# davidesantangelo/krep

Measured on NVIDIA H100. Metric: GB/s scanned (HBM-resident corpus), higher is better.
Workload: dtype u8

## Files before the change

krep_b200/csrc/scan_count.cu:

```cuda
#include <algorithm>
#include "engine.h"
#include "line_rec.cuh"
#include "lit_filters.cuh"

namespace kb {

struct CountDev
{
    LitDevParams p;
    uint64_t own_end;
    uint32_t part_groups, n_parts;
    uint32_t exact;
    uint32_t tail;
    LineRec *recs;
};

struct PartState
{
    uint32_t lines = 0;
    bool has_hit = false, first_open = false, pending = false, seen_nl = false;
    uint64_t covered_to = 0;
};

__device__ __noinline__ unsigned verify_exact_call(const LitDevParams &p, long long cand) { return verify_exact(p, cand); }

__device__ __noinline__ bool scan_for_newline(const LitDevParams &p, uint64_t lo, uint64_t hi)
{
    const uint32_t lane = threadIdx.x & 31;
    if (hi > p.avail_len) hi = p.avail_len;
    for (uint64_t base = lo & ~15ull; base < hi; base += 512)
    {
        const uint64_t unit = base + 16ull * lane;
        uint32_t nm = 0;
        if (unit < hi && unit + 16 > lo)
        {
            if (unit + 16 <= p.avail_len) nm = nl_mask16(__ldg(reinterpret_cast<const uint4 *>(p.text + unit)));
            else
                for (uint64_t q = unit; q < p.avail_len; q++) nm |= (p.text[q] == '\n' ? 1u : 0u) << (uint32_t)(q - unit);
            nm &= range_mask16(unit, lo, hi);
        }
        if (__any_sync(0xffffffffu, nm != 0)) return true;
    }
    return false;
}

__device__ __forceinline__ void settle(const LitDevParams &p, PartState &S, uint64_t upto)
{
    if (S.covered_to < upto && (S.pending || (!S.has_hit && !S.seen_nl)))
        if (scan_for_newline(p, S.covered_to, upto))
        {
            S.pending = false;
            S.seen_nl = true;
        }
}

__device__ __forceinline__ void account(PartState &S, uint32_t hm, uint32_t nm)
{
    const uint32_t lane = threadIdx.x & 31;
    const bool has_nl = nm != 0;
    const uint32_t fnl = has_nl ? (uint32_t)__ffs(nm) - 1 : 0, lnl = has_nl ? 31u - (uint32_t)__clz(nm) : 0;
    const bool f = has_nl && (hm & ((1u << fnl) - 1u)) != 0;
    const bool l = has_nl && ((hm >> lnl) >> 1) != 0;
    uint32_t inner = 0;
    if (__popc(nm) >= 2)
    {
        uint32_t prev = fnl, rest = nm & (nm - 1);
        while (rest)
        {
            const uint32_t nx = (uint32_t)__ffs(rest) - 1;
            if (hm & (((1u << nx) - 1u) & ~((2u << prev) - 1u))) inner++;
            prev = nx;
            rest &= rest - 1;
        }
    }
    const uint32_t A = __ballot_sync(0xffffffffu, has_nl), T = __ballot_sync(0xffffffffu, !has_nl && hm != 0);
    const uint32_t F = __ballot_sync(0xffffffffu, f), Lm = __ballot_sync(0xffffffffu, l);
    uint32_t innersum = 0;
    if (__ballot_sync(0xffffffffu, inner != 0)) innersum = __reduce_add_sync(0xffffffffu, inner);
    if (A == 0)
    {
        if (T)
        {
            if (!S.pending)
            {
                S.lines++;
                if (!S.has_hit && !S.seen_nl) S.first_open = true;
            }
            S.pending = true;
            S.has_hit = true;
        }
        return;
    }
    const uint32_t j1 = (uint32_t)__ffs(A) - 1, jr = 31u - (uint32_t)__clz(A);
    if ((T & ((1u << j1) - 1u)) || ((F >> j1) & 1u))
    {
        if (!S.pending)
        {
            S.lines++;
            if (!S.has_hit && !S.seen_nl) S.first_open = true;
        }
        S.has_hit = true;
    }
    S.pending = false;
    S.seen_nl = true;
    bool gap = false;
    if (has_nl && lane != j1)
    {
        const uint32_t below = A & ((1u << lane) - 1u);
        const uint32_t pj = 31u - (uint32_t)__clz(below);
        const uint32_t between = ((1u << lane) - 1u) & ~((2u << pj) - 1u);
        gap = ((Lm >> pj) & 1u) || (T & between) || f;
    }
    const uint32_t G = __ballot_sync(0xffffffffu, gap);
    S.lines += (uint32_t)__popc(G) + innersum;
    if (G || innersum) S.has_hit = true;
    if (((Lm >> jr) & 1u) || ((T >> jr) >> 1))
    {
        S.lines++;
        S.has_hit = true;
        S.pending = true;
    }
}

__device__ __forceinline__ uint64_t pack_state(const PartState &S)
{
    return (uint64_t)S.lines | ((uint64_t)((S.has_hit ? 1u : 0u) | (S.first_open ? 2u : 0u) | (S.pending ? 4u : 0u) | (S.seen_nl ? 8u : 0u)) << 32);
}
__device__ __forceinline__ void unpack_state(uint64_t k, PartState &S)
{
    S.lines = (uint32_t)k;
    const uint32_t f = (uint32_t)(k >> 32);
    S.has_hit = f & 1u;
    S.first_open = f & 2u;
    S.pending = f & 4u;
    S.seen_nl = f & 8u;
}
__device__ __noinline__ uint64_t account_call(uint64_t packed, uint32_t hm, uint32_t nm)
{
    PartState S;
    unpack_state(packed, S);
    account(S, hm, nm);
    return pack_state(S);
}

template <bool WINDOW>
__device__ __noinline__ uint32_t hit_mask16(const CountDev &D, uint64_t unit, const uint4 &v, uint32_t nx)
{
    const LitDevParams &p = D.p;
    const uint32_t w[5] = {v.x, v.y, v.z, v.w, nx};
    uint32_t hm = 0;
    if (WINDOW)
    {
        const uint32_t mask = p.fold & p.win_mask, k0 = p.K[0];
#pragma unroll
        for (int k = 0; k < 4; k++)
#pragma unroll
            for (int r = 0; r < 4; r++)
            {
                const uint32_t win = r == 0 ? w[k] : __funnelshift_r(w[k], w[k + 1], 8 * r);
                if ((win & mask) == k0)
                {
                    const uint64_t st = unit + 4 * k + r;
                    const bool ok = D.exact ? (st >= p.own_begin && st < p.own_end && st + p.m <= p.avail_len)
                                            : verify_exact_call(p, (long long)st) != 0;
                    if (ok) hm |= 1u << (4 * k + r);
                }
            }
    }
    else
    {
#pragma unroll
        for (int k = 0; k < 4; k++)
#pragma unroll
            for (int d = 0; d < 4; d++)
                if ((w[k] & p.fold) == p.K[d] && verify_exact_call(p, (long long)(unit + 4 * k) - d)) hm |= 1u << (4 * k);
    }
    return hm;
}

__device__ __noinline__ PartState count_tail(const CountDev &D, PartState S, uint64_t cov, uint64_t nl_lo, uint64_t nl_hi, bool window)
{
    const LitDevParams &p = D.p;
    const uint32_t lane = threadIdx.x & 31;
    if (p.avail_len < p.emit_len && cov >= nl_hi) return S;
    const uint64_t last_start = p.avail_len >= p.emit_len ? p.avail_len - p.emit_len : 0;
    uint64_t end = nl_hi > last_start + 1 ? nl_hi : last_start + 1;
    if (!window && end < cov + 1) end = cov + 1;
    for (uint64_t base = cov; base < end; base += 32)
    {
        settle(p, S, base > nl_lo ? base : nl_lo);
        const uint64_t q = base + lane;
        uint32_t hm = 0, nm = 0;
        if (q < end)
        {
            if (p.avail_len >= p.emit_len && q >= p.tail_start && q <= last_start && verify_exact(p, (long long)q)) hm = 1;
            if (!window && q == cov && p.avail_len >= p.emit_len)
                for (uint64_t s = p.tail_start; s < cov && s <= last_start; s++)
                    if (verify_exact(p, (long long)s)) hm = 1;
            if (q >= nl_lo && q < nl_hi && q < p.avail_len && p.text[q] == '\n') nm = 1;
            if (nm) hm = 0;
        }
        account(S, hm, nm);
        S.covered_to = base + 32;
    }
    return S;
}

#ifndef KREP_B200_COUNT_MINB
#define KREP_B200_COUNT_MINB 3
#endif
template <bool WINDOW, bool FOLD, bool MASKED>
__global__ void __launch_bounds__(256, KREP_B200_COUNT_MINB) k_count_lines(const __grid_constant__ CountDev D)
{
    const LitDevParams &p = D.p;
    const uint4 *__restrict__ t4 = reinterpret_cast<const uint4 *>(p.text);
    const uint32_t lane = threadIdx.x & 31;
    const uint32_t warp_global = (blockIdx.x * blockDim.x + threadIdx.x) >> 5, total_warps = (gridDim.x * blockDim.x) >> 5;
    const uint32_t k0 = p.K[0], k1 = p.K[1], k2 = p.K[2], k3 = p.K[3], fold = p.fold, mask = p.win_mask;
    const uint32_t c1 = p.mulc[0], c2 = p.mulc[1], c3 = p.mulc[2];
    for (uint32_t pi = warp_global; pi < D.n_parts; pi += total_warps)
    {
        const uint64_t ga = p.group_begin + (uint64_t)pi * D.part_groups;
        uint64_t gb = ga + D.part_groups;
        if (gb > p.group_end) gb = p.group_end;
        const bool last_part = pi + 1 == D.n_parts;
        const uint64_t nl_lo = ga * 16 > p.own_begin ? ga * 16 : p.own_begin;
        const uint64_t nl_hi = (last_part || gb * 16 > D.own_end) ? D.own_end : gb * 16;
        PartState S;
        S.covered_to = nl_lo;
        for (uint64_t g = ga; g < gb; g += 128)
        {
            uint4 v[4];
            uint32_t nx[4];
            bool ok[4];
#pragma unroll
            for (int u = 0; u < 4; u++)
            {
                const uint64_t gi = g + 32 * u + lane;
                ok[u] = gi < gb;
                v[u] = ok[u] ? ld_stream(t4 + gi) : make_uint4(0u, 0u, 0u, 0u);
                nx[u] = 0;
                if (WINDOW && ok[u] && (lane == 31 || gi + 1 >= gb)) nx[u] = __ldg(reinterpret_cast<const uint32_t *>(t4 + gi + 1));
            }
            uint32_t cand = 0;
#pragma unroll
            for (int u = 0; u < 4; u++)
            {
                bool h;
                if (WINDOW)
                {
                    const uint32_t nb = __shfl_down_sync(0xffffffffu, v[u].x, 1);
                    if (!(lane == 31 || g + 32 * u + lane + 1 >= gb)) nx[u] = nb;
                    h = hit_vec_w<FOLD, MASKED>(v[u], nx[u], fold, mask, k0, c1, c2, c3);
                }
                else
                    h = hit_vec<FOLD>(v[u], fold, k0, k1, k2, k3);
                cand |= (h && ok[u]) ? (1u << u) : 0u;
            }
            const uint32_t any = __reduce_or_sync(0xffffffffu, cand);
            if (any)
            {
                const uint64_t tile_lo = g * 16;
                settle(p, S, tile_lo > nl_lo ? tile_lo : nl_lo);
                const bool inside = tile_lo >= nl_lo && tile_lo + 2048 <= nl_hi;
                uint64_t st = pack_state(S);
#pragma unroll
                for (int u = 0; u < 4; u++)
                {
                    const uint64_t unit = tile_lo + 512ull * u + 16ull * lane;
                    uint32_t hm = 0, nm = 0;
                    if (ok[u])
                    {
                        if ((cand >> u) & 1u) hm = hit_mask16<WINDOW>(D, unit, v[u], nx[u]);
                        nm = nl_mask16(v[u]);
                        if (!inside) nm &= range_mask16(unit, nl_lo, nl_hi);
                    }
                    st = account_call(st, hm, nm);
                }
                unpack_state(st, S);
                S.covered_to = tile_lo + 2048;
            }
        }
        if (last_part && D.tail) S = count_tail(D, S, gb * 16, nl_lo, nl_hi, WINDOW);
        uint32_t flags = 0;
        if (S.has_hit)
        {
            if (S.pending && S.covered_to < nl_hi && scan_for_newline(p, S.covered_to, nl_hi)) S.pending = false;
            flags = LR_HAS_HIT | (S.first_open ? LR_FIRST_OPEN : 0u) | (S.pending ? LR_LAST_PENDING : 0u) | LR_HAS_NL;
        }
        else
        {
            const bool nl = S.seen_nl || (S.covered_to < nl_hi && scan_for_newline(p, S.covered_to, nl_hi));
            flags = nl ? LR_HAS_NL : 0u;
        }
        if (lane == 0) D.recs[pi] = LineRec{S.lines, flags};
    }
}

__global__ void __launch_bounds__(1024) k_count_finish(const LineRec *recs, uint32_t n, uint64_t *d_out, uint64_t *h_out)
{
    __shared__ uint64_t s_lines[1024];
    __shared__ uint32_t s_flags[1024];
    const uint32_t per = (n + blockDim.x - 1) / blockDim.x;
    const uint32_t a = threadIdx.x * per, b = a + per < n ? a + per : n;
    uint64_t lines = 0;
    uint32_t flags = 0;
    for (uint32_t i = a; i < b; i++) append_rec(lines, flags, recs[i].lines, recs[i].flags);
    s_lines[threadIdx.x] = lines;
    s_flags[threadIdx.x] = flags;
    __syncthreads();
    if (threadIdx.x == 0)
    {
        lines = 0;
        flags = 0;
        for (uint32_t t = 0; t < blockDim.x; t++) append_rec(lines, flags, s_lines[t], s_flags[t]);
        d_out[0] = lines;
        d_out[1] = flags;
        h_out[0] = lines;
        h_out[1] = flags;
    }
}

#define CKC(call)                                                                                  \
    do                                                                                             \
    {                                                                                              \
        cudaError_t e_ = (call);                                                                   \
        if (e_ != cudaSuccess)                                                                     \
        {                                                                                          \
            set_error(-2, "CUDA error %s at %s:%d (%s)", cudaGetErrorName(e_), __FILE__, __LINE__, \
                      cudaGetErrorString(e_));                                                     \
            return -2;                                                                             \
        }                                                                                          \
    } while (0)

bool count_lines_eligible(const Plan *plan, const search_params_t *P, int algo)
{
    if (!P->count_lines_mode || plan->is_regex || plan->whole_word == 2) return false;
    if (plan->is_ac)
    {
        for (const std::string &s : plan->patterns)
            if (s.find('\n') != std::string::npos) return false;
        return true;
    }
    if (plan->emit_len != plan->m) return false;
    if (plan->pattern.find('\n') != std::string::npos) return false;
    return algo == KREP_B200_ALGO_BMH || algo == KREP_B200_ALGO_KMP || algo == KREP_B200_ALGO_MEMCHR ||
           algo == KREP_B200_ALGO_MEMCHR_SHORT || algo == KREP_B200_ALGO_SSE42;
}

int ensure_line_out(DevCtx &E, uint64_t n)
{
    if (n <= E.line_out_cap) return 0;
    CKC(cudaDeviceSynchronize());
    cudaFree(E.d_line_out);
    cudaFreeHost(E.h_line_out);
    E.d_line_out = nullptr;
    E.h_line_out = nullptr;
    E.line_out_cap = 0;
    uint64_t cap = 64;
    while (cap < n) cap *= 2;
    CKC(cudaMalloc(&E.d_line_out, cap * 2 * sizeof(uint64_t)));
    CKC(cudaHostAlloc(&E.h_line_out, cap * 2 * sizeof(uint64_t), cudaHostAllocMapped | cudaHostAllocPortable));
    E.line_out_cap = cap;
    return 0;
}

int launch_count_lines(DevCtx &E, const Plan *plan, const krep_b200_shard_t *sh, cudaStream_t stream, uint64_t index)
{
    if (((uintptr_t)sh->d_text & 15) != 0)
    {
        set_error(-3, "shard text pointer must be 16-byte aligned");
        return -3;
    }
    const PlanDev *pd = plan_on_device(plan, E);
    if (!pd) return -2;
    if (ensure_line_out(E, index + 1) != 0) return -2;
    if (plan->is_ac)
    {
        const int slot = set_count_slot(E);
        const int rc = set_count_begin(E, plan, sh, stream, slot);
        return rc != 0 ? rc : set_count_end(E, plan, sh, stream, slot, index);
    }
    CountDev D;
    memset(&D, 0, sizeof D);
    LitDevParams &p = D.p;
    const uint64_t own_end = sh->own_end < sh->avail_len ? sh->own_end : sh->avail_len;
    p.text = (const uint8_t *)sh->d_text;
    p.avail_len = sh->avail_len;
    p.own_begin = sh->own_begin;
    p.own_end = own_end;
    p.global_offset = sh->global_offset;
    p.prev_byte = sh->prev_byte;
    p.next_byte = sh->next_byte;
    uint64_t total_groups;
    const bool window = plan->filter == FILTER_WINDOW4;
    if (!window)
    {
        total_groups = sh->avail_len / 16;
        p.tail_start = total_groups ? total_groups * 16 - 3 : 0;
    }
    else
    {
        total_groups = sh->avail_len >= 20 ? (sh->avail_len - 20) / 16 + 1 : 0;
        p.tail_start = total_groups * 16;
    }
    p.group_begin = sh->own_begin / 16;
    p.group_end = (own_end + 2) / 16 + 1;
    D.tail = p.group_end > total_groups ? 1u : 0u;
    if (p.group_end > total_groups) p.group_end = total_groups;
    if (p.group_begin > p.group_end) p.group_begin = p.group_end;
    p.m = plan->m;
    p.emit_len = plan->emit_len;
    for (int d = 0; d < 4; d++) p.K[d] = plan->K[d];
    p.fold = plan->fold;
    p.win_mask = plan->win_mask;
    p.mulc[0] = 1u << 24;
    p.mulc[1] = 1u << 16;
    p.mulc[2] = 1u << 8;
    p.pat_val = pd->d_pat_val;
    p.pat_mask = pd->d_pat_mask;
    p.whole_word = plan->whole_word;
    D.own_end = own_end;
    {
        bool letters = true;
        for (unsigned char ch : plan->pattern) letters &= is_alpha_c(ch);
        D.exact = (window && plan->m <= 4 && plan->whole_word == 0 && (plan->case_sensitive || letters)) ? 1u : 0u;
    }
    const uint64_t groups = p.group_end - p.group_begin;
    const char *v = getenv("KREP_B200_COUNT_PART_KB");
    const uint32_t kb_ = v && atoi(v) > 0 ? (uint32_t)atoi(v) : 64;
    uint64_t part = std::max<uint32_t>(128, kb_ * 64 / 128 * 128);
    const uint64_t max_parts = 1u << 18;
    if ((groups + part - 1) / part > max_parts) part = ((groups + max_parts - 1) / max_parts + 127) / 128 * 128;
    D.part_groups = (uint32_t)part;
    D.n_parts = (uint32_t)std::max<uint64_t>((groups + part - 1) / part, 1);
    if (D.n_parts > E.line_recs_cap)
    {
        CKC(cudaStreamSynchronize(stream));
        cudaFree(E.d_line_recs);
        E.d_line_recs = nullptr;
        E.line_recs_cap = 0;
        const uint64_t cap = std::max<uint64_t>(D.n_parts, 1u << 16);
        CKC(cudaMalloc(&E.d_line_recs, cap * sizeof(LineRec)));
        E.line_recs_cap = cap;
    }
    D.recs = (LineRec *)E.d_line_recs;
    const bool folded = plan->fold != 0xFFFFFFFFu, masked = plan->win_mask != 0xFFFFFFFFu;
    const uint64_t want_blocks = ((uint64_t)D.n_parts + 7) / 8;
    const unsigned grid = (unsigned)std::min<uint64_t>(want_blocks, (uint64_t)E.sm_count * KREP_B200_COUNT_MINB);
    if (!window)
    {
        if (folded) k_count_lines<false, true, false><<<grid, 256, 0, stream>>>(D);
        else k_count_lines<false, false, false><<<grid, 256, 0, stream>>>(D);
    }
    else if (folded)
    {
        if (masked) k_count_lines<true, true, true><<<grid, 256, 0, stream>>>(D);
        else k_count_lines<true, true, false><<<grid, 256, 0, stream>>>(D);
    }
    else
    {
        if (masked) k_count_lines<true, false, true><<<grid, 256, 0, stream>>>(D);
        else k_count_lines<true, false, false><<<grid, 256, 0, stream>>>(D);
    }
    CKC(cudaGetLastError());
    k_count_finish<<<1, 1024, 0, stream>>>(D.recs, D.n_parts, E.d_line_out + 2 * index, E.h_line_out + 2 * index);
    CKC(cudaGetLastError());
    count_launch(2);
    return 0;
}

uint64_t combine_line_records(const uint64_t *recs, size_t n)
{
    uint64_t lines = 0;
    uint32_t flags = 0;
    for (size_t i = 0; i < n; i++) append_rec(lines, flags, recs[2 * i], (uint32_t)recs[2 * i + 1]);
    return lines;
}

}
```

Baseline: 3124.

## Stage count-kernel tiles through cp.async shared-memory ring with per-lane line records

Rewrites the line-counting kernel so each warp streams 2 KB tiles through a 4-stage cp.async shared-memory ring, and each lane handles 64 contiguous bytes instead of strided 16-byte units. The sequential warp-wide account/settle state machine and the separate newline rescans are replaced by per-lane bitmask line records combined with a shuffle-based append_rec reduction. The special tail pass goes away because the last tile is zero-padded. Blocks shrink to 4 warps and the occupancy hint rises to 4. The aim is to hide HBM latency and cut serial per-tile bookkeeping, at the cost of shared-memory footprint and more complex boundary handling.

```diff
diff --git a/krep_b200/csrc/scan_count.cu b/krep_b200/csrc/scan_count.cu
--- a/krep_b200/csrc/scan_count.cu
+++ b/krep_b200/csrc/scan_count.cu
@@ -11,290 +11,211 @@
     uint64_t own_end;
     uint32_t part_groups, n_parts;
     uint32_t exact;
-    uint32_t tail;
     LineRec *recs;
 };
 
-struct PartState
-{
-    uint32_t lines = 0;
-    bool has_hit = false, first_open = false, pending = false, seen_nl = false;
-    uint64_t covered_to = 0;
-};
-
-__device__ __noinline__ unsigned verify_exact_call(const LitDevParams &p, long long cand) { return verify_exact(p, cand); }
-
-__device__ __noinline__ bool scan_for_newline(const LitDevParams &p, uint64_t lo, uint64_t hi)
-{
-    const uint32_t lane = threadIdx.x & 31;
-    if (hi > p.avail_len) hi = p.avail_len;
-    for (uint64_t base = lo & ~15ull; base < hi; base += 512)
-    {
-        const uint64_t unit = base + 16ull * lane;
-        uint32_t nm = 0;
-        if (unit < hi && unit + 16 > lo)
+constexpr uint32_t COUNT_WARPS = 4;
+constexpr uint32_t COUNT_STAGES = 4;
+constexpr uint32_t COUNT_STAGE_BYTES = 2048 + 16;
+#ifndef KREP_B200_COUNT_MINB
+#define KREP_B200_COUNT_MINB 4
+#endif
+
+template <uint32_t UNITS>
+__device__ __forceinline__ void stage_tile(uint32_t s_dst, const uint8_t *text, uint64_t avail, uint64_t pos, uint32_t lane)
+{
+#pragma unroll
+    for (uint32_t i = 0; i < (UNITS + 31) / 32; i++)
+    {
+        const uint32_t u = lane + 32 * i;
+        if (u >= UNITS) break;
+        const uint64_t b = pos + 16ull * u;
+        const uint32_t n = b >= avail ? 0u : (avail - b >= 16 ? 16u : (uint32_t)(avail - b));
+        const uint8_t *src = n ? text + b : text;
+        asm volatile("cp.async.cg.shared.global [%0], [%1], 16, %2;" ::"r"(s_dst + 16u * u), "l"(src), "r"(n) : "memory");
+    }
+    asm volatile("cp.async.commit_group;" ::: "memory");
+}
+
+__device__ __forceinline__ uint64_t umin64(uint64_t a, uint64_t b) { return a < b ? a : b; }
+
+__device__ __forceinline__ uint64_t range_mask64(uint64_t base, uint64_t lo, uint64_t hi)
+{
+    uint64_t m = ~0ull;
+    if (base < lo) m = lo - base >= 64 ? 0ull : m << (uint32_t)(lo - base);
+    if (base + 64 > hi) m = hi <= base ? 0ull : m & (~0ull >> (uint32_t)(64 - (hi - base)));
+    return m;
+}
+
+template <bool WINDOW>
+__device__ __forceinline__ uint32_t cand16(const LitDevParams &p, const uint4 &v, uint32_t nx)
+{
+    const uint32_t w[5] = {v.x, v.y, v.z, v.w, nx};
+    uint32_t c = 0;
+#pragma unroll
+    for (int k = 0; k < 4; k++)
+#pragma unroll
+        for (int r = 0; r < 4; r++)
         {
-            if (unit + 16 <= p.avail_len) nm = nl_mask16(__ldg(reinterpret_cast<const uint4 *>(p.text + unit)));
+            bool h;
+            if (WINDOW)
+            {
+                const uint32_t win = r == 0 ? w[k] : __funnelshift_r(w[k], w[k + 1], 8 * r);
+                h = (win & (p.fold & p.win_mask)) == p.K[0];
+            }
             else
-                for (uint64_t q = unit; q < p.avail_len; q++) nm |= (p.text[q] == '\n' ? 1u : 0u) << (uint32_t)(q - unit);
-            nm &= range_mask16(unit, lo, hi);
+                h = (w[k] & p.fold) == p.K[r];
+            c |= (h ? 1u : 0u) << (4 * k + r);
         }
-        if (__any_sync(0xffffffffu, nm != 0)) return true;
-    }
-    return false;
-}
-
-__device__ __forceinline__ void settle(const LitDevParams &p, PartState &S, uint64_t upto)
-{
-    if (S.covered_to < upto && (S.pending || (!S.has_hit && !S.seen_nl)))
-        if (scan_for_newline(p, S.covered_to, upto))
-        {
-            S.pending = false;
-            S.seen_nl = true;
-        }
-}
-
-__device__ __forceinline__ void account(PartState &S, uint32_t hm, uint32_t nm)
-{
-    const uint32_t lane = threadIdx.x & 31;
-    const bool has_nl = nm != 0;
-    const uint32_t fnl = has_nl ? (uint32_t)__ffs(nm) - 1 : 0, lnl = has_nl ? 31u - (uint32_t)__clz(nm) : 0;
-    const bool f = has_nl && (hm & ((1u << fnl) - 1u)) != 0;
-    const bool l = has_nl && ((hm >> lnl) >> 1) != 0;
-    uint32_t inner = 0;
-    if (__popc(nm) >= 2)
-    {
-        uint32_t prev = fnl, rest = nm & (nm - 1);
-        while (rest)
-        {
-            const uint32_t nx = (uint32_t)__ffs(rest) - 1;
-            if (hm & (((1u << nx) - 1u) & ~((2u << prev) - 1u))) inner++;
-            prev = nx;
-            rest &= rest - 1;
-        }
-    }
-    const uint32_t A = __ballot_sync(0xffffffffu, has_nl), T = __ballot_sync(0xffffffffu, !has_nl && hm != 0);
-    const uint32_t F = __ballot_sync(0xffffffffu, f), Lm = __ballot_sync(0xffffffffu, l);
-    uint32_t innersum = 0;
-    if (__ballot_sync(0xffffffffu, inner != 0)) innersum = __reduce_add_sync(0xffffffffu, inner);
-    if (A == 0)
-    {
-        if (T)
-        {
-            if (!S.pending)
-            {
-                S.lines++;
-                if (!S.has_hit && !S.seen_nl) S.first_open = true;
-            }
-            S.pending = true;
-            S.has_hit = true;
-        }
-        return;
-    }
-    const uint32_t j1 = (uint32_t)__ffs(A) - 1, jr = 31u - (uint32_t)__clz(A);
-    if ((T & ((1u << j1) - 1u)) || ((F >> j1) & 1u))
-    {
-        if (!S.pending)
-        {
-            S.lines++;
-            if (!S.has_hit && !S.seen_nl) S.first_open = true;
-        }
-        S.has_hit = true;
-    }
-    S.pending = false;
-    S.seen_nl = true;
-    bool gap = false;
-    if (has_nl && lane != j1)
-    {
-        const uint32_t below = A & ((1u << lane) - 1u);
-        const uint32_t pj = 31u - (uint32_t)__clz(below);
-        const uint32_t between = ((1u << lane) - 1u) & ~((2u << pj) - 1u);
-        gap = ((Lm >> pj) & 1u) || (T & between) || f;
-    }
-    const uint32_t G = __ballot_sync(0xffffffffu, gap);
-    S.lines += (uint32_t)__popc(G) + innersum;
-    if (G || innersum) S.has_hit = true;
-    if (((Lm >> jr) & 1u) || ((T >> jr) >> 1))
-    {
-        S.lines++;
-        S.has_hit = true;
-        S.pending = true;
-    }
-}
-
-__device__ __forceinline__ uint64_t pack_state(const PartState &S)
-{
-    return (uint64_t)S.lines | ((uint64_t)((S.has_hit ? 1u : 0u) | (S.first_open ? 2u : 0u) | (S.pending ? 4u : 0u) | (S.seen_nl ? 8u : 0u)) << 32);
-}
-__device__ __forceinline__ void unpack_state(uint64_t k, PartState &S)
-{
-    S.lines = (uint32_t)k;
-    const uint32_t f = (uint32_t)(k >> 32);
-    S.has_hit = f & 1u;
-    S.first_open = f & 2u;
-    S.pending = f & 4u;
-    S.seen_nl = f & 8u;
-}
-__device__ __noinline__ uint64_t account_call(uint64_t packed, uint32_t hm, uint32_t nm)
-{
-    PartState S;
-    unpack_state(packed, S);
-    account(S, hm, nm);
-    return pack_state(S);
-}
-
-template <bool WINDOW>
-__device__ __noinline__ uint32_t hit_mask16(const CountDev &D, uint64_t unit, const uint4 &v, uint32_t nx)
-{
+    return c;
+}
+
+__device__ __forceinline__ void lane_record(uint64_t H, uint64_t N, uint32_t &lines, uint32_t &flags)
+{
+    lines = 0;
+    flags = N ? LR_HAS_NL : 0u;
+    if (H)
+    {
+        const uint64_t t = ~N + H;
+        const bool open = t < H;
+        lines = (uint32_t)__popcll(t & N) + (open ? 1u : 0u);
+        flags = LR_HAS_HIT | LR_HAS_NL | ((H & ((N & (0ull - N)) - 1ull)) ? LR_FIRST_OPEN : 0u) |
+                (open ? LR_LAST_PENDING : 0u);
+    }
+}
+
+template <bool WINDOW, bool FOLD, bool MASKED>
+__global__ void __launch_bounds__(32 * COUNT_WARPS, KREP_B200_COUNT_MINB) k_count_lines(const __grid_constant__ CountDev D)
+{
+    constexpr uint32_t UNITS = WINDOW ? 129 : 128;
+    __shared__ __align__(16) uint8_t s_ring[COUNT_WARPS][COUNT_STAGES][COUNT_STAGE_BYTES];
     const LitDevParams &p = D.p;
-    const uint32_t w[5] = {v.x, v.y, v.z, v.w, nx};
-    uint32_t hm = 0;
-    if (WINDOW)
-    {
-        const uint32_t mask = p.fold & p.win_mask, k0 = p.K[0];
-#pragma unroll
-        for (int k = 0; k < 4; k++)
-#pragma unroll
-            for (int r = 0; r < 4; r++)
-            {
-                const uint32_t win = r == 0 ? w[k] : __funnelshift_r(w[k], w[k + 1], 8 * r);
-                if ((win & mask) == k0)
-                {
-                    const uint64_t st = unit + 4 * k + r;
-                    const bool ok = D.exact ? (st >= p.own_begin && st < p.own_end && st + p.m <= p.avail_len)
-                                            : verify_exact_call(p, (long long)st) != 0;
-                    if (ok) hm |= 1u << (4 * k + r);
-                }
-            }
-    }
-    else
-    {
-#pragma unroll
-        for (int k = 0; k < 4; k++)
-#pragma unroll
-            for (int d = 0; d < 4; d++)
-                if ((w[k] & p.fold) == p.K[d] && verify_exact_call(p, (long long)(unit + 4 * k) - d)) hm |= 1u << (4 * k);
-    }
-    return hm;
-}
-
-__device__ __noinline__ PartState count_tail(const CountDev &D, PartState S, uint64_t cov, uint64_t nl_lo, uint64_t nl_hi, bool window)
-{
-    const LitDevParams &p = D.p;
-    const uint32_t lane = threadIdx.x & 31;
-    if (p.avail_len < p.emit_len && cov >= nl_hi) return S;
-    const uint64_t last_start = p.avail_len >= p.emit_len ? p.avail_len - p.emit_len : 0;
-    uint64_t end = nl_hi > last_start + 1 ? nl_hi : last_start + 1;
-    if (!window && end < cov + 1) end = cov + 1;
-    for (uint64_t base = cov; base < end; base += 32)
-    {
-        settle(p, S, base > nl_lo ? base : nl_lo);
-        const uint64_t q = base + lane;
-        uint32_t hm = 0, nm = 0;
-        if (q < end)
-        {
-            if (p.avail_len >= p.emit_len && q >= p.tail_start && q <= last_start && verify_exact(p, (long long)q)) hm = 1;
-            if (!window && q == cov && p.avail_len >= p.emit_len)
-                for (uint64_t s = p.tail_start; s < cov && s <= last_start; s++)
-                    if (verify_exact(p, (long long)s)) hm = 1;
-            if (q >= nl_lo && q < nl_hi && q < p.avail_len && p.text[q] == '\n') nm = 1;
-            if (nm) hm = 0;
-        }
-        account(S, hm, nm);
-        S.covered_to = base + 32;
-    }
-    return S;
-}
-
-#ifndef KREP_B200_COUNT_MINB
-#define KREP_B200_COUNT_MINB 3
-#endif
-template <bool WINDOW, bool FOLD, bool MASKED>
-__global__ void __launch_bounds__(256, KREP_B200_COUNT_MINB) k_count_lines(const __grid_constant__ CountDev D)
-{
-    const LitDevParams &p = D.p;
-    const uint4 *__restrict__ t4 = reinterpret_cast<const uint4 *>(p.text);
-    const uint32_t lane = threadIdx.x & 31;
-    const uint32_t warp_global = (blockIdx.x * blockDim.x + threadIdx.x) >> 5, total_warps = (gridDim.x * blockDim.x) >> 5;
+    const uint32_t lane = threadIdx.x & 31, warp = threadIdx.x >> 5;
+    const uint32_t warp_global = blockIdx.x * COUNT_WARPS + warp, total_warps = gridDim.x * COUNT_WARPS;
     const uint32_t k0 = p.K[0], k1 = p.K[1], k2 = p.K[2], k3 = p.K[3], fold = p.fold, mask = p.win_mask;
     const uint32_t c1 = p.mulc[0], c2 = p.mulc[1], c3 = p.mulc[2];
+    const uint32_t ring = (uint32_t)__cvta_generic_to_shared(&s_ring[warp][0][0]);
+    const uint32_t rot = (lane >> 1) & 3;
+    const uint64_t s_lo = p.own_begin, s_hi = p.avail_len >= p.m ? umin64(D.own_end, p.avail_len - p.m + 1) : 0;
+
+    uint32_t ld_pi = warp_global;
+    uint64_t ld_g = p.group_begin + (uint64_t)ld_pi * D.part_groups;
+    auto stage_next = [&](uint32_t slot) {
+        while (ld_pi < D.n_parts && ld_g >= umin64(p.group_begin + (uint64_t)ld_pi * D.part_groups + D.part_groups, p.group_end))
+        {
+            ld_pi += total_warps;
+            ld_g = p.group_begin + (uint64_t)ld_pi * D.part_groups;
+        }
+        if (ld_pi < D.n_parts)
+        {
+            stage_tile<UNITS>(ring + slot * COUNT_STAGE_BYTES, p.text, p.avail_len, ld_g * 16, lane);
+            ld_g += 128;
+        }
+        else
+            asm volatile("cp.async.commit_group;" ::: "memory");
+    };
+#pragma unroll
+    for (uint32_t s = 0; s + 1 < COUNT_STAGES; s++) stage_next(s);
+
+    uint32_t seq = 0;
     for (uint32_t pi = warp_global; pi < D.n_parts; pi += total_warps)
     {
         const uint64_t ga = p.group_begin + (uint64_t)pi * D.part_groups;
-        uint64_t gb = ga + D.part_groups;
-        if (gb > p.group_end) gb = p.group_end;
+        const uint64_t gb = umin64(ga + D.part_groups, p.group_end);
         const bool last_part = pi + 1 == D.n_parts;
         const uint64_t nl_lo = ga * 16 > p.own_begin ? ga * 16 : p.own_begin;
         const uint64_t nl_hi = (last_part || gb * 16 > D.own_end) ? D.own_end : gb * 16;
-        PartState S;
-        S.covered_to = nl_lo;
-        for (uint64_t g = ga; g < gb; g += 128)
+        uint32_t lines = 0, flags = 0;
+        for (uint64_t g = ga; g < gb; g += 128, seq++)
         {
-            uint4 v[4];
-            uint32_t nx[4];
-            bool ok[4];
-#pragma unroll
-            for (int u = 0; u < 4; u++)
-            {
-                const uint64_t gi = g + 32 * u + lane;
-                ok[u] = gi < gb;
-                v[u] = ok[u] ? ld_stream(t4 + gi) : make_uint4(0u, 0u, 0u, 0u);
-                nx[u] = 0;
-                if (WINDOW && ok[u] && (lane == 31 || gi + 1 >= gb)) nx[u] = __ldg(reinterpret_cast<const uint32_t *>(t4 + gi + 1));
+            asm volatile("cp.async.wait_group %0;" ::"n"(COUNT_STAGES - 2) : "memory");
+            __syncwarp();
+            stage_next((seq + COUNT_STAGES - 1) % COUNT_STAGES);
+            const uint8_t *tile = &s_ring[warp][seq % COUNT_STAGES][0];
+            const uint64_t tile_lo = g * 16, base = tile_lo + 64ull * lane;
+            uint4 q[4];
+            uint32_t sh[4];
+#pragma unroll
+            for (int k = 0; k < 4; k++)
+            {
+                const uint32_t slot = (k + rot) & 3;
+                q[k] = *reinterpret_cast<const uint4 *>(tile + 64 * lane + 16 * slot);
+                sh[k] = 16 * slot;
+            }
+            uint32_t nx[4] = {0, 0, 0, 0};
+            if (WINDOW)
+            {
+                const uint32_t f0 = rot == 0 ? q[0].x : rot == 1 ? q[3].x : rot == 2 ? q[2].x : q[1].x;
+                uint32_t nl = __shfl_down_sync(0xffffffffu, f0, 1);
+                if (lane == 31) nl = *reinterpret_cast<const uint32_t *>(tile + 2048);
+#pragma unroll
+                for (int k = 0; k < 4; k++) nx[k] = sh[k] == 48 ? nl : q[(k + 1) & 3].x;
             }
             uint32_t cand = 0;
 #pragma unroll
-            for (int u = 0; u < 4; u++)
-            {
-                bool h;
-                if (WINDOW)
+            for (int k = 0; k < 4; k++)
+            {
+                const bool h = WINDOW ? hit_vec_w<FOLD, MASKED>(q[k], nx[k], fold, mask, k0, c1, c2, c3)
+                                      : hit_vec<FOLD>(q[k], fold, k0, k1, k2, k3);
+                cand |= (h ? 1u : 0u) << k;
+            }
+            bool tile_hit = false;
+            uint64_t H = 0;
+            if (__any_sync(0xffffffffu, cand != 0))
+            {
+                uint64_t C = 0;
+#pragma unroll
+                for (int k = 0; k < 4; k++)
+                    if ((cand >> k) & 1u) C |= (uint64_t)cand16<WINDOW>(p, q[k], nx[k]) << sh[k];
+                if (WINDOW && D.exact)
                 {
-                    const uint32_t nb = __shfl_down_sync(0xffffffffu, v[u].x, 1);
-                    if (!(lane == 31 || g + 32 * u + lane + 1 >= gb)) nx[u] = nb;
-                    h = hit_vec_w<FOLD, MASKED>(v[u], nx[u], fold, mask, k0, c1, c2, c3);
+                    H = C;
+                    if (!(tile_lo >= s_lo && tile_lo + 2048 <= s_hi)) H &= range_mask64(base, s_lo, s_hi);
                 }
                 else
-                    h = hit_vec<FOLD>(v[u], fold, k0, k1, k2, k3);
-                cand |= (h && ok[u]) ? (1u << u) : 0u;
-            }
-            const uint32_t any = __reduce_or_sync(0xffffffffu, cand);
-            if (any)
-            {
-                const uint64_t tile_lo = g * 16;
-                settle(p, S, tile_lo > nl_lo ? tile_lo : nl_lo);
-                const bool inside = tile_lo >= nl_lo && tile_lo + 2048 <= nl_hi;
-                uint64_t st = pack_state(S);
-#pragma unroll
-                for (int u = 0; u < 4; u++)
+                    while (C)
+                    {
+                        const uint32_t j = (uint32_t)__ffsll((long long)C) - 1, at = WINDOW ? j : (j & ~3u);
+                        C &= C - 1;
+                        if (verify_exact(p, (long long)(base + at) - (long long)(j - at))) H |= 1ull << at;
+                    }
+                tile_hit = __any_sync(0xffffffffu, H != 0);
+            }
+            const bool need_nl = tile_hit || (flags & LR_LAST_PENDING) || flags == 0;
+            if (need_nl)
+            {
+                uint64_t N = 0;
+#pragma unroll
+                for (int k = 0; k < 4; k++) N |= (uint64_t)nl_mask16(q[k]) << sh[k];
+                if (!(tile_lo >= nl_lo && tile_lo + 2048 <= nl_hi)) N &= range_mask64(base, nl_lo, nl_hi);
+                uint32_t rl, rf;
+                if (tile_hit)
                 {
-                    const uint64_t unit = tile_lo + 512ull * u + 16ull * lane;
-                    uint32_t hm = 0, nm = 0;
-                    if (ok[u])
+                    lane_record(H, N, rl, rf);
+#pragma unroll
+                    for (uint32_t off = 1; off < 32; off <<= 1)
                     {
-                        if ((cand >> u) & 1u) hm = hit_mask16<WINDOW>(D, unit, v[u], nx[u]);
-                        nm = nl_mask16(v[u]);
-                        if (!inside) nm &= range_mask16(unit, nl_lo, nl_hi);
+                        const uint32_t ol = __shfl_down_sync(0xffffffffu, rl, off), of = __shfl_down_sync(0xffffffffu, rf, off);
+                        uint64_t l64 = rl;
+                        append_rec(l64, rf, ol, of);
+                        rl = (uint32_t)l64;
                     }
-                    st = account_call(st, hm, nm);
+                    rl = __shfl_sync(0xffffffffu, rl, 0);
+                    rf = __shfl_sync(0xffffffffu, rf, 0);
                 }
-                unpack_state(st, S);
-                S.covered_to = tile_lo + 2048;
+                else
+                {
+                    rl = 0;
+                    rf = __any_sync(0xffffffffu, N != 0) ? LR_HAS_NL : 0u;
+                }
+                uint64_t l64 = lines;
+                append_rec(l64, flags, rl, rf);
+                lines = (uint32_t)l64;
             }
         }
-        if (last_part && D.tail) S = count_tail(D, S, gb * 16, nl_lo, nl_hi, WINDOW);
-        uint32_t flags = 0;
-        if (S.has_hit)
-        {
-            if (S.pending && S.covered_to < nl_hi && scan_for_newline(p, S.covered_to, nl_hi)) S.pending = false;
-            flags = LR_HAS_HIT | (S.first_open ? LR_FIRST_OPEN : 0u) | (S.pending ? LR_LAST_PENDING : 0u) | LR_HAS_NL;
-        }
-        else
-        {
-            const bool nl = S.seen_nl || (S.covered_to < nl_hi && scan_for_newline(p, S.covered_to, nl_hi));
-            flags = nl ? LR_HAS_NL : 0u;
-        }
-        if (lane == 0) D.recs[pi] = LineRec{S.lines, flags};
-    }
+        if (lane == 0) D.recs[pi] = LineRec{lines, flags};
+    }
+    asm volatile("cp.async.wait_all;" ::: "memory");
 }
 
 __global__ void __launch_bounds__(1024) k_count_finish(const LineRec *recs, uint32_t n, uint64_t *d_out, uint64_t *h_out)
@@ -392,22 +313,10 @@
     p.global_offset = sh->global_offset;
     p.prev_byte = sh->prev_byte;
     p.next_byte = sh->next_byte;
-    uint64_t total_groups;
+    const uint64_t total_groups = (sh->avail_len + 15) / 16;
     const bool window = plan->filter == FILTER_WINDOW4;
-    if (!window)
-    {
-        total_groups = sh->avail_len / 16;
-        p.tail_start = total_groups ? total_groups * 16 - 3 : 0;
-    }
-    else
-    {
-        total_groups = sh->avail_len >= 20 ? (sh->avail_len - 20) / 16 + 1 : 0;
-        p.tail_start = total_groups * 16;
-    }
     p.group_begin = sh->own_begin / 16;
-    p.group_end = (own_end + 2) / 16 + 1;
-    D.tail = p.group_end > total_groups ? 1u : 0u;
-    if (p.group_end > total_groups) p.group_end = total_groups;
+    p.group_end = std::min<uint64_t>((own_end + 2) / 16 + 1, total_groups);
     if (p.group_begin > p.group_end) p.group_begin = p.group_end;
     p.m = plan->m;
     p.emit_len = plan->emit_len;
@@ -446,22 +355,23 @@
     }
     D.recs = (LineRec *)E.d_line_recs;
     const bool folded = plan->fold != 0xFFFFFFFFu, masked = plan->win_mask != 0xFFFFFFFFu;
-    const uint64_t want_blocks = ((uint64_t)D.n_parts + 7) / 8;
+    const uint64_t want_blocks = ((uint64_t)D.n_parts + COUNT_WARPS - 1) / COUNT_WARPS;
     const unsigned grid = (unsigned)std::min<uint64_t>(want_blocks, (uint64_t)E.sm_count * KREP_B200_COUNT_MINB);
+    const unsigned threads = 32 * COUNT_WARPS;
     if (!window)
     {
-        if (folded) k_count_lines<false, true, false><<<grid, 256, 0, stream>>>(D);
-        else k_count_lines<false, false, false><<<grid, 256, 0, stream>>>(D);
+        if (folded) k_count_lines<false, true, false><<<grid, threads, 0, stream>>>(D);
+        else k_count_lines<false, false, false><<<grid, threads, 0, stream>>>(D);
     }
     else if (folded)
     {
-        if (masked) k_count_lines<true, true, true><<<grid, 256, 0, stream>>>(D);
-        else k_count_lines<true, true, false><<<grid, 256, 0, stream>>>(D);
+        if (masked) k_count_lines<true, true, true><<<grid, threads, 0, stream>>>(D);
+        else k_count_lines<true, true, false><<<grid, threads, 0, stream>>>(D);
     }
     else
     {
-        if (masked) k_count_lines<true, false, true><<<grid, 256, 0, stream>>>(D);
-        else k_count_lines<true, false, false><<<grid, 256, 0, stream>>>(D);
+        if (masked) k_count_lines<true, false, true><<<grid, threads, 0, stream>>>(D);
+        else k_count_lines<true, false, false><<<grid, threads, 0, stream>>>(D);
     }
     CKC(cudaGetLastError());
     k_count_finish<<<1, 1024, 0, stream>>>(D.recs, D.n_parts, E.d_line_out + 2 * index, E.h_line_out + 2 * index);
```

Result: no change. 3123, median of 6 (-0.0%).
